# souravc83/Blackbox-Coresets-VI

Hardware: AMD Instinct MI355X
Metric: ELBO inner-steps/sec (S MC samples x M pseudopoints) at 1/2/4/8 GPU (higher is better)
Workload: dtype f32; 1 GPU; C3 fn2 full-cov MLP 64-40-40-2, S=128, M=100, one GPU (BASELINE configs[2]); S_total=128, M=100, D=64, H=40, C=2, params=4730326, parallelism=one GPU, adam=robust_higher DifferentiableAdam, elbo_finite=True

## Files before the change

### blackbox-coresets-vi_amd/csrc/capi.cpp

```cpp
#include <algorithm>
#include <cmath>
#include <cstdio>
#include <cstring>
#include <mutex>
#include <string>
#include <vector>

#include "psvi_diag.h"
#include "psvi_internal.hpp"

namespace psvi {
Diag g_diag;
}

using namespace psvi;

namespace {

thread_local std::string g_err;

int fail(int code, const std::string& msg) {
    g_err = msg;
    return code;
}
// ... 24 lines not shown
        if (d->dims[l] < 1) return fail(PSVI_EINVAL, "layer dims must be >= 1");
    if (d->S < 1) return fail(PSVI_EINVAL, "S must be >= 1");
    if (d->M < 1) return fail(PSVI_EINVAL, "M must be >= 1");
    if (!(d->prior_sd > 0.f)) return fail(PSVI_EINVAL, "prior_sd must be > 0");
    return 0;
}

int plan_to_device(psvi_plan& p) {
    const int S = p.d.S;
    const bool fullcov = p.family == PSVI_FAMILY_FULLCOV;
    if (int rc = upload(p.fwd)) return rc;
    if (int rc = upload(p.frb)) return rc;
    if (int rc = upload(p.upd)) return rc;
    if (p.fwd.n() > 0 && !p.fwd_part.alloc(sizeof(float) * (size_t)p.fwd.n() * S * kFwdRows))
        return fail(PSVI_EUNSUP, "cannot allocate the sample-phase scratch");
    if (p.fuse_sample && p.n_uslots > 0) {
        if (int rc = upload(p.ufrb)) return rc;
        if (!p.upd_part.alloc(sizeof(float) * (size_t)p.n_uslots * S * 64))
            return fail(PSVI_EUNSUP, "cannot allocate the fused-sample scratch");
    }
    if (p.str.n() > 0) {
        if (int rc = upload(p.str)) return rc;
        if (int rc = upload(p.sfrb)) return rc;
        const size_t nb = (size_t)std::max(1, p.sfrb.n());
        if (!p.str_part.alloc(sizeof(float) * (size_t)p.n_sslots * S * 64) ||
            !p.str_cnt.alloc(sizeof(int) * nb, true) || !p.str_bms.alloc(sizeof(float) * 128 * nb))
            return fail(PSVI_EUNSUP, "cannot allocate the streaming-update scratch");
    }
    if (p.n_kwg() > 0) {
        if (int rc = upload(p.ks_tiles)) return rc;
        if (int rc = upload(p.ks_segs)) return rc;
        if (int rc = upload(p.ks_off)) return rc;
        if (!p.ks_slots.alloc(sizeof(float) * (size_t)std::max(1, p.n_ks_slots) * kKsSlotFloats) ||
            !p.ks_cnt.alloc(sizeof(int) * std::max(1, p.n_ks_cnt), true))
            return fail(PSVI_EUNSUP, "cannot allocate the K-split update's slots");
    }
    if (p.n_fswg() > 0) {
        if (int rc = upload(p.fs_segs)) return rc;
        if (int rc = upload(p.fs_off)) return rc;
        if (int rc = upload(p.fs_rb)) return rc;
        if (int rc = upload(p.fp_segs)) return rc;
        if (int rc = upload(p.fp_off)) return rc;
        if (int rc = upload(p.fp_rb)) return rc;
        if (!p.fs_part.alloc(sizeof(float) * (size_t)std::max({1, p.n_fs_slots, p.n_fp_slots}) *
                             kKsPass * kFwdRows))
            return fail(PSVI_EUNSUP, "cannot allocate the segmented sample's slots");
    }
    if (fullcov) {
        net_xmap(p, p.xmap.host, p.net_bands.host);
        if (int rc = upload(p.xmap)) return rc;
        if (int rc = upload(p.net_bands)) return rc;
    }
    if (fullcov && p.mchunks > 1 &&
        !p.net_slots.alloc(sizeof(float) * (size_t)p.mchunks * std::max(1, p.s_cnt[p.rank]) * p.n_tot))
        return fail(PSVI_EUNSUP, "cannot allocate the network's pseudopoint-chunk slots");
    if (p.family == PSVI_FAMILY_MEANFIELD &&
        !p.mf_slots.alloc(sizeof(float) * (size_t)std::max(1, p.s_cnt[p.rank]) * p.mchunks * p.n_tot))
        return fail(PSVI_EUNSUP, "cannot allocate the mean-field gradient slots");
    if (fullcov && p.fuse_sample && p.tiles_total > 0 && !p.aux.create())
        return fail(PSVI_EUNSUP, "cannot create the inner loop's conversion stream");
    if (p.eps_planes_ok) {
        p.eps_planes_tab.host.assign(1, p.eps_planes);
        if (int rc = upload(p.eps_planes_tab)) return rc;
    }
    if (p.family == PSVI_FAMILY_LENET && !p.lenet_scratch.alloc(lenet_ws(p, nullptr).bytes))
        return fail(PSVI_EUNSUP, "cannot allocate the LeNet activation scratch");
    return 0;
}

hipStream_t as_stream(void* s) { return reinterpret_cast<hipStream_t>(s); }

int g_loop_every = 0;
std::vector<hipEvent_t> g_loop_ev[2];

void loop_events_clear() {
    for (auto& v : g_loop_ev) {
        for (hipEvent_t e : v) (void)hipEventDestroy(e);
        v.clear();
    }
}

hipError_t loop_event(int k, hipStream_t st) {
    hipEvent_t e;
    const hipError_t rc = hipEventCreate(&e);
    if (rc != hipSuccess) return rc;
    g_loop_ev[k].push_back(e);
    return hipEventRecord(e, st);
}

}

// ... 15 lines not shown
        case PSVI_DBG_FWD_ABLATION: g_diag.fwd_ablation = value; return 0;
        case PSVI_DBG_UPD_CHUNK: g_plan_dbg.upd_chunk_tiles = value; return 0;
        case PSVI_DBG_UPD_STREAM_OFF: g_diag.stream_off = value; return 0;
        case PSVI_DBG_STREAM_BF_OFF: g_diag.stream_bf_off = value; return 0;
        case PSVI_DBG_KSTREAM_OFF: g_diag.ks_off = value; return 0;
        case PSVI_DBG_KSTREAM_WGS: g_plan_dbg.ks_wgs = value; return 0;
        case PSVI_DBG_FWD_SEG_OFF: g_diag.fs_off = value; return 0;
        case PSVI_DBG_FWD_SEG_BF_OFF: g_diag.fs_bf_off = value; return 0;
        case PSVI_DBG_FWD_PAIR_BF: g_diag.fwd_pair_bf = value; return 0;
        case PSVI_DBG_STREAM_FOLD_OFF: g_diag.stream_fold_off = value; return 0;
        case PSVI_DBG_KSTREAM_BF_OFF: g_diag.ks_bf_off = value; return 0;
        case PSVI_DBG_ROP_VALU: g_diag.rop_valu = value; return 0;
        case PSVI_DBG_NET_SCALAR_LOADS: g_diag.net_scalar_loads = value; return 0;
        case PSVI_DBG_NET_MLOOP_OFF: g_diag.net_mloop_off = value; return 0;
        case PSVI_DBG_NET_GEO_OFF: g_diag.net_geo_off = value; return 0;
        case PSVI_DBG_NET_DRAW_SPARE_OFF: g_diag.net_draw_spare_off = value; return 0;
        case PSVI_DBG_NET_DRAW_ROLE1:
            if (value < 0 || value > 32) return fail(PSVI_EINVAL, "0..32");
            g_diag.net_draw_role1 = value;
            return 0;
        case PSVI_DBG_STREAM_WGS: g_plan_dbg.stream_wgs = value; return 0;
        case PSVI_DBG_STREAM_COST: g_plan_dbg.stream_cost = value; return 0;
        case PSVI_DBG_STREAM_RR: g_plan_dbg.stream_rr = value; return 0;
        case PSVI_DBG_LENET_ABLATION: g_diag.lenet_abl = value; return 0;
        case PSVI_DBG_NET_THREADS:
            if (value != 0 && value != 256 && value != 512) return fail(PSVI_EINVAL, "256 or 512");
            g_diag.net_threads = value;
            return 0;
        default: return fail(PSVI_EINVAL, "unknown debug key");
    }
}

int psvi_debug_loop_timing(double* out) {
    if (!out) return fail(PSVI_EINVAL, "null out");
    for (int k = 0; k < 2; ++k) {
        double sum = 0.0;
        const auto& v = g_loop_ev[k];
        for (size_t i = 0; i + 1 < v.size(); i += 2) {
            float ms = 0.f;
            HIP_TRY(hipEventSynchronize(v[i + 1]));
            HIP_TRY(hipEventElapsedTime(&ms, v[i], v[i + 1]));
            sum += ms;
        }
        const size_t n = v.size() / 2;
        out[k] = n ? 1e3 * sum / (double)n : 0.0;
        if (k == 0) out[2] = (double)n;
// ... 23 lines not shown
        return fail(PSVI_EINVAL, "unknown family");
    psvi_net_desc dl;
    if (family == PSVI_FAMILY_LENET && d) {
        dl = *d;
        dl.n_layers = 5;
        const int dims[6] = {784, 6, 16, 120, 84, 10};
        for (int l = 0; l < 6; ++l) dl.dims[l] = dims[l];
        d = &dl;
    }
    if (int rc = check_desc(d)) return rc;
    if (world < 1 || world > kMaxWorld || rank < 0 || rank >= world)
        return fail(PSVI_EINVAL, "world/rank out of range (world <= 8)");
    int ndev = 0;
    const bool have_dev = hipGetDeviceCount(&ndev) == hipSuccess && ndev > 0;
    if (have_dev) {
        static std::once_flag once;
        std::call_once(once, net_set_lds_limit);
    }
    psvi_plan* p = new psvi_plan();
    p->family = family;
    p->d = *d;
    p->world = world;
    p->rank = rank;
    std::string err;
    int rc = build_plan(*p, err);
    if (rc) rc = fail(rc, err);
    if (!rc && have_dev) {
        rc = plan_to_device(*p);
        p->on_device = rc == 0;
    }
    if (rc) {
        psvi_plan_destroy(p);
        return rc;
    }
    *out = p;
    return 0;
}

int psvi_plan_create_lik(int32_t family, const psvi_net_desc* d, int32_t world, int32_t rank,
                         const psvi_likelihood* lik, psvi_plan** out) {
    if (!lik || lik->kind == PSVI_LIK_CATEGORICAL)
        return psvi_plan_create(family, d, world, rank, out);
    if (!out) return fail(PSVI_EINVAL, "null out");
    *out = nullptr;
    if (lik->kind != PSVI_LIK_GAUSSIAN && lik->kind != PSVI_LIK_BERNOULLI)
        return fail(PSVI_EINVAL, "unknown likelihood kind");
// ... 1247 lines not shown
```

### blackbox-coresets-vi_amd/csrc/kernels_mvn_stream.hip

```cpp
#include "mvn_common.hpp"

namespace psvi {

struct StrArgs {
    const StreamRange* ranges;
    int nb[kMaxL];
    const float* eps;
    const float* eps_next;
    const float* g;
    int ldg, S;
    int64_t g_total, e_total;
    float* params;
    float* m;
    float* v;
    float* tp;
    float* tm;
    float* tv;
    float* part;
    double* kl_out;
    int include_kl;
    unsigned long long* stamps;
    float inv_s0sq, log_s0;
    AdamC adam;
    int xcol[kMaxL];
    MvnLayerArgs lay[kMaxL];
    const uint16_t* ep;
    const uint16_t* enp;
    int64_t pl;
// ... 44 lines not shown
        d = __builtin_elementwise_fma(sq, f32x2{a.inv_sqrt_bc2, a.inv_sqrt_bc2}, f32x2{a.eps, a.eps});
        const f32x2 r = {__builtin_amdgcn_rcpf(d[0]), __builtin_amdgcn_rcpf(d[1])};
        return p - (f32x2{a.lr_bc1, a.lr_bc1} * m) * r;
    } else {
        v = __builtin_elementwise_fma(b2, v, (omb2 * g) * g) + f32x2{1e-12f, 1e-12f};
        const f32x2 vb = v * f32x2{a.inv_bc2, a.inv_bc2};
        d = f32x2{__builtin_amdgcn_sqrtf(vb[0]), __builtin_amdgcn_sqrtf(vb[1])} + f32x2{a.eps, a.eps};
        const f32x2 r = {__builtin_amdgcn_rcpf(d[0]), __builtin_amdgcn_rcpf(d[1])};
        return p - f32x2{a.lr, a.lr} * (m * f32x2{a.inv_bc1, a.inv_bc1}) * r;
    }
}

template <int NS, int KIND, bool DIAG = false, bool SC1 = true, bool PAD = false>
__global__ __launch_bounds__(256, 1) void mvn_stream_kernel(StrArgs a) {
    constexpr int KT = 16 * NS;
    __shared__ __attribute__((aligned(16))) f32x4 sm[4 * kStrBuf + 2048];
    f32x4* const Gl4 = sm + 4 * kStrBuf;
    const float* const Gl = reinterpret_cast<const float*>(Gl4);
    const int tid = threadIdx.x, lane = tid & 63, wv = wave_id();
    const int wr = wv >> 1, wc = wv & 1, h = lane >> 5, l32 = lane & 31;
    const StreamRange R = a.ranges[blockIdx.x];
    const int t0 = __builtin_amdgcn_readfirstlane(R.t0);
    const int t1 = __builtin_amdgcn_readfirstlane(R.t1);
    int slot = __builtin_amdgcn_readfirstlane(R.slot0);
    const int S = a.S;
    unsigned long long tph[10] = {0, 0, 0, 0, 0, 0, 0, 0, 0, 0}, tlast = 0;
    auto ph = [&](int q) __attribute__((always_inline)) {
        if (DIAG && tid == 0) {
            const unsigned long long tt = __builtin_amdgcn_s_memtime();
            if (q >= 0) tph[q] += tt - tlast;
            tlast = tt;
        }
    };
    const int e_hi = PAD ? 0x7fffffff : (int)a.e_total - 4;
    const int g_hi = PAD ? 0x7fffffff : (int)a.g_total - 4;
    constexpr int SMAX = 32 * NS - 1;

    f32x4 ereg[8], enreg[8];
    auto load_E = [&](const StrTile& T) __attribute__((always_inline)) {
#pragma unroll
        for (int j = 0; j < 8; ++j) {
            const int f = tid + 256 * j, s = min(f >> 4, SMAX), c4 = f & 15;
            const int off = min(T.eoff + s * T.n + 64 * T.k + 4 * c4, e_hi);
            ereg[j] = *reinterpret_cast<const f32x4*>(a.eps + off);
            enreg[j] = *reinterpret_cast<const f32x4*>(a.eps_next + off);
        }
    };
// ... 66 lines not shown
#pragma unroll
        for (int q = 0; q < 16; ++q) xacc[sb][q] = 0.f;
    float klp = 0.f, kld = 0.f;
    f32x2 kl2 = {0.f, 0.f};

    int okd[8];
    {
        const int c = 32 * wc + l32, c4 = c >> 2;
#pragma unroll
        for (int k = 0; k < 8; ++k) okd[k] = h * 64 + 4 * ((c4 ^ h) ^ (2 * k)) + (c & 3);
    }
    int okx[4];
#pragma unroll
    for (int g = 0; g < 4; ++g) okx[g] = l32 * 16 + ((8 * wc + 2 * g + h) ^ (l32 & 15));
    const int ogb = h * 64 + 32 * wr + l32;

    if (DIAG && tid == 0) {
        a.stamps[(size_t)blockIdx.x * 16 + 12] = __builtin_amdgcn_s_memtime();
        a.stamps[(size_t)blockIdx.x * 16 + 13] = __builtin_amdgcn_s_memrealtime();
    }
    int tl = __builtin_amdgcn_readfirstlane(R.lbk0 >> 28);
    int tb_ = __builtin_amdgcn_readfirstlane((R.lbk0 >> 14) & 0x3fff);
    int tk = __builtin_amdgcn_readfirstlane(R.lbk0 & 0x3fff);
    StrTile cur = str_tile(a, tl, tb_, tk);
    load_E(cur);
    load_G(cur);
    store_E(0, cur);
    store_G(cur);
    __syncthreads();

    auto tile = [&](int i, const StrTile& nxt, auto has_next_c, auto newband_c) __attribute__((always_inline)) {
        constexpr bool has_next = decltype(has_next_c)::value;
        constexpr bool newband = decltype(newband_c)::value;
        const int bi = (i - t0) & 1;
        ph(-1);
        const float* Ef = reinterpret_cast<const float*>(sm + 2 * bi * kStrBuf);
        const f32x4* En = sm + (2 * bi + 1) * kStrBuf;
        load_pmv(cur);
        floatx16 acc;
#pragma unroll
        for (int q = 0; q < 16; ++q) acc[q] = 0.f;
#pragma unroll
        for (int t = 0; t < KT; ++t)
            acc = __builtin_amdgcn_mfma_f32_32x32x2f32(Ef[okd[t & 7] + 128 * t], Gl[ogb + 128 * t],
                                                       acc, 0, 0, 0);
        ph(0);
        const int n = cur.n, r = 64 * cur.b + 32 * wr + l32;
        if (cur.k == cur.b && wc == 0) {
            const int c = 32 * wr + l32;
            float pm2[2], ps2[2];
#pragma unroll
            for (int ww = 0; ww < 2; ++ww) {
                const int w = 2 * h + ww;
                float gm = 0.f, gsum = 0.f;
#pragma unroll
                for (int hh = 0; hh < (NS > 2 ? 2 : 1); ++hh)
#pragma unroll
// ... 106 lines not shown
#pragma unroll
                for (int q = 0; q < NLOAD; ++q)
                    if ((q * NSLOT) / (NLOAD > 0 ? NLOAD : 1) == k) issue_load(q);
                __builtin_amdgcn_sched_barrier(0x6);
            }
        }
        ph(2);
        ph(3);
        ph(4);
        if constexpr (has_next) store_E(bi ^ 1, nxt);
        ph(5);
        if constexpr (!has_next || newband) {
            __syncthreads();
            float* X = reinterpret_cast<float*>(sm + 2 * bi * kStrBuf);
            if (wc == 1) {
#pragma unroll
                for (int sb = 0; sb < NS; ++sb)
#pragma unroll
                    for (int q = 0; q < 16; ++q) X[((wr * NS + sb) * 16 + q) * 64 + lane] = xacc[sb][q];
            }
            if constexpr (newband) store_G(nxt);
            __syncthreads();
            if (wc == 0) {
                float* dst = a.part + (size_t)slot * S * 64 + 32 * wr + l32;
#pragma unroll
                for (int sb = 0; sb < NS; ++sb)
#pragma unroll
                    for (int q = 0; q < 16; ++q) {
                        const int s = 32 * sb + (q & 3) + 8 * (q >> 2) + 4 * h;
                        dst[(size_t)s * 64] = xacc[sb][q] + X[((wr * NS + sb) * 16 + q) * 64 + lane];
                    }
            }
#pragma unroll
            for (int sb = 0; sb < NS; ++sb)
#pragma unroll
                for (int q = 0; q < 16; ++q) xacc[sb][q] = 0.f;
            ++slot;
        }
        ph(6);
        __syncthreads();
        ph(7);
        if (DIAG && tid == 0) ++tph[9];
    };
    using T_ = std::true_type;
    using F_ = std::false_type;
    for (int i = t0; i + 1 < t1; ++i) {
        if (++tk > tb_) {
            tk = 0;
            int nbl = a.nb[0];
#pragma unroll
            for (int l = 1; l < kMaxL; ++l)
                if (tl == l) nbl = a.nb[l];
            if (++tb_ == nbl) {
                tb_ = 0;
                ++tl;
            }
        }
        const StrTile nxt = str_tile(a, tl, tb_, tk);
        if (nxt.l != cur.l || nxt.b != cur.b)
            tile(i, nxt, T_{}, T_{});
        else
            tile(i, nxt, T_{}, F_{});
        cur = nxt;
    }
    tile(t1 - 1, cur, F_{}, F_{});
    if (DIAG && tid == 0) {
        unsigned long long* o = a.stamps + (size_t)blockIdx.x * 16;
#pragma unroll
        for (int q = 0; q < 10; ++q) o[q] = tph[q];
        o[10] = __builtin_amdgcn_s_memtime();
        o[11] = __builtin_amdgcn_s_memrealtime();
    }
    klp = (klp + (kl2[0] + kl2[1])) * (0.5f * a.inv_s0sq) + kld;
    if (a.kl_out && a.include_kl) {
        const float tot = block_sum(klp, reinterpret_cast<float*>(sm));
        if (tid == 0) atomicAdd(a.kl_out, (double)tot);
    }
}


template <int KIND, bool DIAG = false, bool FOLD = false>
__global__ __launch_bounds__(512, 1) void mvn_stream_bf2_kernel(StrArgs a) {
    __shared__ __attribute__((aligned(16))) uint8_t smb[9 * kBfImg];
    uint8_t* const Eb = smb;
    uint8_t* const Gb = smb + 3 * kBfImg;
    uint8_t* const En = smb + 6 * kBfImg;
    float* const Xs = reinterpret_cast<float*>(En);
    float* const Xd = reinterpret_cast<float*>(Eb);
    uint32_t* const Xl = reinterpret_cast<uint32_t*>(Eb + 16384);
    float* const Xg = reinterpret_cast<float*>(Eb + 40960);
    typedef unsigned u32x4 __attribute__((ext_vector_type(4)));
    typedef unsigned u32x2 __attribute__((ext_vector_type(2)));
    const int tid = threadIdx.x, lane = tid & 63, wv = wave_id();
    const int q = wv & 3, hk = wv >> 2, wr = q >> 1, wc = q & 1, h = lane >> 5, l32 = lane & 31;
    const int pw = wv ^ 4;
    const StreamRange R = a.ranges[blockIdx.x];
    const int t0 = __builtin_amdgcn_readfirstlane(R.t0);
    const int t1 = __builtin_amdgcn_readfirstlane(R.t1);
    int slot = __builtin_amdgcn_readfirstlane(R.slot0);
    const int S = a.S;
    unsigned long long tph[11] = {0, 0, 0, 0, 0, 0, 0, 0, 0, 0, 0}, tlast = 0;
    if (DIAG && tid == 0) a.stamps[(size_t)blockIdx.x * 16 + 13] = __builtin_amdgcn_s_memtime();
    auto ph = [&](int qq) __attribute__((always_inline)) {
        if (DIAG && wv == 0) {
            const unsigned long long tt = __builtin_amdgcn_s_memtime();
            if (qq >= 0) tph[qq] += tt - tlast;
            tlast = tt;
        }
    };

    u32x4 stg[6];
    const int srow0 = tid >> 3, ch = tid & 7;
    const int st_col = srow0 * 128 + ((ch ^ (((srow0 >> 1) & 1) << 2)) << 4);
    const int st_row0 = img_row(srow0, 8 * ch), st_row1 = img_row(srow0, 8 * ch + 4);
    auto store_col = [&]() __attribute__((always_inline)) {
#pragma unroll
        for (int j = 0; j < 6; ++j)
            *reinterpret_cast<u32x4*>(Eb + st_col + (j >> 1) * kBfImg + 8192 * (j & 1)) = stg[j];
    };
    auto store_row = [&]() __attribute__((always_inline)) {
#pragma unroll
        for (int j = 0; j < 6; ++j) {
// ... 33 lines not shown
        return __builtin_bit_cast(u32x4, __builtin_amdgcn_raw_buffer_load_b128(r, vo, so, 0));
    };
    auto load_G = [&](const StrTile& T, int j) __attribute__((always_inline)) {
        const int so = __builtin_amdgcn_readfirstlane(4 * (32 * j * a.ldg + T.xc + 64 * T.b));
        greg[j] = __builtin_bit_cast(f32x4, ldb(rs_g, vo_g, so));
    };
    floatx16 xacc[2];
#pragma unroll
    for (int j = 0; j < 2; ++j)
#pragma unroll
        for (int qq = 0; qq < 16; ++qq) xacc[j][qq] = 0.f;
    float kld = 0.f;
    f32x2 kl2 = {0.f, 0.f};
    const int g16 = lane >> 4, qq4 = (lane >> 2) & 3, pp = lane & 3;
    const int ca = 32 * wc + 16 * (g16 & 1) + 4 * pp;
    const int cg = 32 * wr + 16 * (g16 & 1) + 4 * pp;
    const uint8_t* const rda = Eb + img_col(8 * h + qq4, ca);
    const uint8_t* const rdb = Gb + img_col(8 * h + qq4, cg);
    const int xsw = (l32 >> 1) & 7;

    int tl = __builtin_amdgcn_readfirstlane(R.lbk0 >> 28);
    int tb_ = __builtin_amdgcn_readfirstlane((R.lbk0 >> 14) & 0x3fff);
    int tk = __builtin_amdgcn_readfirstlane(R.lbk0 & 0x3fff);
    StrTile cur = str_tile(a, tl, tb_, tk);
    {
        const uint32_t vo = vo_planes(cur);
#pragma unroll
        for (int j = 0; j < 4; ++j) load_G(cur, j);
#pragma unroll
        for (int j = 0; j < 6; ++j) stg[j] = ldb(rs_e, vo, so_planes(cur, j));
        store_col();
#pragma unroll
        for (int j = 0; j < 6; ++j) stg[j] = ldb(rs_en, vo, so_planes(cur, j));
        store_row();
        split_G();
    }
    __syncthreads();

    auto issue_a = [&](int qi, const StrTile& nxt, bool has_next, uint32_t vo_n) __attribute__((always_inline)) {
        if (qi < 6) {
            const int gi = qi / 3, which = qi % 3;
            const int so = __builtin_amdgcn_readfirstlane((int)(cur.tb * 4));
            const u32x4 x = __builtin_bit_cast(
                u32x4, __builtin_amdgcn_raw_buffer_load_b128(rs_t, vo_f + 1024 * gi,
                                                             which == 0 ? so : which == 1 ? so + tmb : so + tvb,
                                                             PSVI_STATE_LOAD_AUX));
// ... 80 lines not shown
            }
#pragma unroll
            for (int i = 0; i < KR; ++i)
                if (k0 + i < nk)
#pragma unroll
                    for (int m = 0; m < 4; ++m) A[m][i & 3] += v[m][i];
        }
#pragma unroll
        for (int m = 0; m < 4; ++m) {
            const f32x4 t = (A[m][0] + A[m][1]) + (A[m][2] + A[m][3]);
            const int rr = 32 * (m >> 1) + lt;
            if (rr < R) {
#pragma unroll
                for (int e = 0; e < 4; ++e)
                    a.x[(int64_t)smp(m, e) * a.ldx + xcol + rr] =
                        (mu[m >> 1] + mul_unfused(dg[m >> 1], ev[m][e])) + t[e];
            }
        }
    };

    auto tile = [&](const StrTile& nxt, auto has_next_c, auto newband_c) __attribute__((always_inline)) {
        constexpr bool has_next = decltype(has_next_c)::value;
        constexpr bool newband = decltype(newband_c)::value;
        ph(-1);
        const bool diag = cur.k == cur.b && wc == wr;
        const uint32_t vo_n = vo_planes(nxt);
        floatx16 acc;
#pragma unroll
        for (int qq = 0; qq < 16; ++qq) acc[qq] = 0.f;
        float dgm = 0.f, dgs = 0.f;
        auto read_ab = [&](int t, bf8v (&av)[3], bf8v (&bv)[3]) __attribute__((always_inline)) {
#pragma unroll
            for (int p = 0; p < 3; ++p) {
                typedef __attribute__((address_space(3))) s4v* lds_s4;
                const int o = p * kBfImg + 2048 * t;
                av[p] = cat44(__builtin_amdgcn_ds_read_tr16_b64_v4i16((lds_s4)(rda + o)),
                              __builtin_amdgcn_ds_read_tr16_b64_v4i16((lds_s4)(rda + o + 512)));
                bv[p] = cat44(__builtin_amdgcn_ds_read_tr16_b64_v4i16((lds_s4)(rdb + o)),
                              __builtin_amdgcn_ds_read_tr16_b64_v4i16((lds_s4)(rdb + o + 512)));
            }
        };
#pragma unroll
        for (int t = 0; t < 4; ++t) {
            bf8v fa[3], fb[3];
            read_ab(4 * hk + t, fa, fb);
#pragma unroll
// ... 177 lines not shown
                            for (int e = 0; e < 4; ++e)
                                v4[e] = __float_as_uint(xacc[j][4 * qg + e] +
                                                        Xs[(((wr * 2 + hk) * 2 + j) * 16 + 4 * qg + e) * 64 + lane]);
                            BSTORE128(v4, rs_p, (uint32_t)((((((wr * 2 + hk) * 2 + j) * 4 + qg) * 64 + lane)) * 16),
                                      sob, 16);
                        }
                } else {
                    const uint32_t vb = (uint32_t)((32 * wr + l32 + 64 * (64 * hk + 4 * h)) * 4);
#pragma unroll
                    for (int j = 0; j < 2; ++j)
#pragma unroll
                        for (int qq = 0; qq < 16; ++qq) {
                            const int sl = 32 * j + (qq & 3) + 8 * (qq >> 2);
                            const float v = xacc[j][qq] + Xs[(((wr * 2 + hk) * 2 + j) * 16 + qq) * 64 + lane];
                            __builtin_amdgcn_raw_buffer_store_b32(__builtin_bit_cast(int, v), rs_p,
                                                                  vb + (uint32_t)(sl * 256), sob, 0);
                        }
                }
            }
#pragma unroll
            for (int j = 0; j < 2; ++j)
#pragma unroll
                for (int qq = 0; qq < 16; ++qq) xacc[j][qq] = 0.f;
            ++slot;
            if constexpr (FOLD) band_arrive();
        }
        ph(6);
        __syncthreads();
        ph(7);
        if constexpr (has_next) store_row();
        if constexpr (newband) {
            split_G();
            __syncthreads();
        }
        ph(8);
        if (DIAG && wv == 0) ++tph[9];
    };
    using T_ = std::true_type;
    using F_ = std::false_type;
    for (int i = t0; i + 1 < t1; ++i) {
        if (++tk > tb_) {
            tk = 0;
            int nbl = a.nb[0];
#pragma unroll
            for (int l = 1; l < kMaxL; ++l)
                if (tl == l) nbl = a.nb[l];
            if (++tb_ == nbl) {
                tb_ = 0;
                ++tl;
            }
        }
        const StrTile nxt = str_tile(a, tl, tb_, tk);
        if (nxt.l != cur.l || nxt.b != cur.b)
            tile(nxt, T_{}, T_{});
        else
            tile(nxt, T_{}, F_{});
        cur = nxt;
    }
    tile(cur, F_{}, F_{});
    if constexpr (FOLD) {
        ph(-1);
        for (int i = 0; i < nfold; ++i) band_combine(__builtin_amdgcn_readfirstlane(fold_list[i]));
        ph(10);
    }
    if (DIAG && tid == 0) {
        unsigned long long* o = a.stamps + (size_t)blockIdx.x * 16;
#pragma unroll
        for (int qq = 0; qq < 10; ++qq) o[qq] = tph[qq];
        o[10] = __builtin_amdgcn_s_memtime();
        o[11] = __builtin_amdgcn_s_memrealtime();
        o[12] = tph[10];
    }
// ... 14 lines not shown
    if (KIND == PSVI_ADAM_HIGHER && diag)
        hipLaunchKernelGGL((mvn_stream_kernel<4, PSVI_ADAM_HIGHER, true>), g, bl, 0, st, b);
    else if (pad)
        hipLaunchKernelGGL((mvn_stream_kernel<4, KIND, false, true, true>), g, bl, 0, st, b);
    else
        hipLaunchKernelGGL((mvn_stream_kernel<4, KIND>), g, bl, 0, st, b);
}
template <int KIND>
static void launch_stream_bf(bool diag, bool fold, dim3 g, hipStream_t st, const StrArgs& b) {
    const dim3 bl(512);
    if (KIND == PSVI_ADAM_HIGHER && diag && fold)
        hipLaunchKernelGGL((mvn_stream_bf2_kernel<PSVI_ADAM_HIGHER, true, true>), g, bl, 0, st, b);
    else if (fold)
        hipLaunchKernelGGL((mvn_stream_bf2_kernel<KIND, false, true>), g, bl, 0, st, b);
    else
        hipLaunchKernelGGL(mvn_stream_bf2_kernel<KIND>, g, bl, 0, st, b);
}

hipError_t launch_mvn_stream(const psvi_plan& p, const MvnUpdate& r, hipStream_t st) {
    StrArgs b{};
    fill_update(p, r, b);
    const int64_t tf = p.tiles_total * 4096;
    b.ranges = p.str.dev;
    b.eps_next = r.next.eps;
    b.tp = r.tstate;
    b.tm = r.tstate + tf;
    b.tv = r.tstate + 2 * tf;
    b.part = p.str_part.dev;
    for (int l = 0; l < p.L; ++l) {
        b.xcol[l] = p.xcol_l[p.rank][l];
        b.nb[l] = p.lay[l].nb;
    }
    const dim3 sg(p.str.n());
    const bool higher = b.adam.kind == PSVI_ADAM_HIGHER;
    const bool bf = r.eps_planes && r.next.planes && p.bf_stream && r.padded && !g_diag.stream_bf_off;
    if (bf) {
        b.stamps = g_diag.bf_stamps;
        b.ep = r.eps_planes;
        b.enp = r.next.planes;
        b.pl = p.eps_planes.pl;
        for (int l = 0; l < p.L; ++l) {
            b.ppoff[l] = p.eps_planes.poff[l];
            b.npad[l] = p.eps_planes.npad[l];
        }
        const bool fold = p.str_cnt.dev && p.str_bms.dev && p.str_max_ends <= kFoldMax && !g_diag.stream_fold_off;
        b.rbs = p.sfrb.dev;
// ... 17 lines not shown
```

### blackbox-coresets-vi_amd/csrc/plan_tables.cpp

```cpp
#include <algorithm>
#include <string>
#include <vector>

#include "psvi_internal.hpp"

namespace psvi {

PlanDebug g_plan_dbg;

namespace {

constexpr int kFwdKChunk = 256;
constexpr int64_t kLenetRowFloats = 2 * 1176 + 400 * 2 + 120 * 2 + 84 * 2 + 10;
constexpr int64_t kMaxOff = (int64_t(1) << 31) - 4096;

int fail(std::string& err, int code, const char* msg) {
    err = msg;
    return code;
}

std::vector<int64_t> cut_runs(const std::vector<double>& cum, int nwg) {
    const int64_t U = (int64_t)cum.size() - 1;
    std::vector<int64_t> cut(nwg + 1, 0);
    cut[nwg] = U;
// ... 131 lines not shown
            p.frb.host.push_back(
                FwdRowBlock{slot0, (int)fwd.size() - slot0, r1 - r0, xc + (r0 - lo), l, r0});
        }
        for (int b = lo / 64; 64 * b < hi; ++b) {
            const int slot0 = nslots;
            for (int k0 = 0; k0 <= b; k0 += ch) {
                const int k1 = std::min(b + 1, k0 + ch);
                upd.push_back(UpdChunk{l, 64 * b, k0, k1, lo, hi, xc - lo, k1 == b + 1, nslots++});
            }
            const int r0 = std::max(64 * b, lo), r1 = std::min(64 * b + 64, hi);
            p.ufrb.host.push_back(FwdRowBlock{slot0, nslots - slot0, r1 - r0, xc + (r0 - lo), l, r0});
        }
    }
    std::stable_sort(fwd.begin(), fwd.end(), [](const FwdItem& a, const FwdItem& b) {
        return (a.k1 - a.k0) > (b.k1 - b.k0);
    });
    p.upd.host = xcd_order(upd);
    p.n_uslots = nslots;
    p.upd_tiles = tiles;
}

void build_stream(psvi_plan& p) {
    const int r = p.rank;
    std::vector<uint32_t> tmap;
    std::vector<int> tband;
    int nband = 0;
    for (int l = 0; l < p.L; ++l)
        for (int b = 0; b < p.lay[l].nb; ++b, ++nband)
            for (int k = 0; k <= b; ++k) {
                tmap.push_back((uint32_t)l << 28 | (uint32_t)b << 14 | (uint32_t)k);
                tband.push_back(nband);
            }
    const int T = (int)tmap.size();
    const int nwg = std::max(1, std::min(g_plan_dbg.stream_wgs > 0 ? g_plan_dbg.stream_wgs : 256, T));
    const int cost = g_plan_dbg.stream_cost;
    std::vector<double> cum(T + 1, 0.0);
    for (int t = 0; t < T; ++t) {
        const uint32_t k = tmap[t] & 0x3fff, b = (tmap[t] >> 14) & 0x3fff;
        const double wd = cost >= 0 ? (cost / 1000) * 0.01 : 1.5;
        const double wf = cost >= 0 ? (cost % 1000) * 0.01 : 1.0;
        cum[t + 1] = cum[t] + 1.0 + (k == b ? wd : 0.0) + (k == 0 ? wf : 0.0);
    }
    const std::vector<int64_t> cut = cut_runs(cum, nwg);
    std::vector<StreamRange> runs;
    std::vector<std::vector<int>> band_slots(nband);
    int ns = 0;
    for (int w = 0; w < nwg; ++w) {
        const int t0 = (int)cut[w], t1 = (int)cut[w + 1];
        runs.push_back(StreamRange{t0, t1, ns, t0 < T ? tmap[t0] : 0u});
        int ends = 0;
        for (int t = t0; t < t1; ++t)
            if (t == t0 || tband[t] != tband[t - 1]) {
                band_slots[tband[t]].push_back(ns++);
                ++ends;
            }
        p.str_max_ends = std::max(p.str_max_ends, ends);
    }
    int bid = 0;
    for (int l = 0; l < p.L; ++l)
        for (int b = 0; b < p.lay[l].nb; ++b, ++bid) {
            const int r0 = 64 * b, R = std::min(64, p.lay[l].n - r0);
            const auto& sl = band_slots[bid];
            p.sfrb.host.push_back(
                FwdRowBlock{sl.front(), (int)sl.size(), R, p.xcol_l[r][l] + r0, l, r0});
        }
    for (int w = 0; w < nwg; ++w)
        p.str.host.push_back(runs[g_plan_dbg.stream_rr ? w : xcd_run(w, nwg)]);
    p.n_sslots = ns;
}

void build_kstream(psvi_plan& p) {
    const int r = p.rank, np = (p.d.S + kKsPass - 1) / kKsPass;
    std::vector<KsTile>& tiles = p.ks_tiles.host;
    tiles.clear();
    for (const ShardRun& run : p.runs[r])
        for (int b = run.lo / 64; 64 * b < run.hi; ++b)
            for (int k = 0; k <= b; ++k)
                tiles.push_back(KsTile{run.layer, 64 * b, k, k == b, 64 * b,
                                       std::min(64 * b + 64, p.lay[run.layer].n), run.col - run.lo, -1});
    const int T = (int)tiles.size();
    std::vector<KsSeg>& segs = p.ks_segs.host;
    std::vector<int>& off = p.ks_off.host;
    segs.clear();
    off.clear();
    p.n_ks_slots = p.n_ks_cnt = 0;
    if (T == 0) return;
    const int64_t U = (int64_t)T * np;
    int nwg = (int)std::min<int64_t>(U, g_plan_dbg.ks_wgs > 0 ? g_plan_dbg.ks_wgs : 512);
    if (nwg >= 8) nwg -= nwg % 8;
    std::vector<double> cum(U + 1, 0.0);
    for (int64_t u = 0; u < U; ++u) cum[u + 1] = cum[u] + 1.0 + (u % np == np - 1 ? 0.5 : 0.0);
// ... 225 lines not shown
```

### blackbox-coresets-vi_amd/csrc/psvi_diag.h

```cpp
#ifndef PSVI_DIAG_H
#define PSVI_DIAG_H
#include <stdint.h>

#ifdef __cplusplus
extern "C" {
#endif

#define PSVI_DBG_NET_ABLATION 1
int psvi_debug_set(int32_t key, int32_t value);
#define PSVI_DBG_NET_STAMPS 2
#define PSVI_DBG_UPD_ABLATION 3
#define PSVI_DBG_UPD_STAMPS 4
#define PSVI_DBG_NET_SPLIT_BELOW 5
#define PSVI_DBG_FWD_ABLATION 6
#define PSVI_DBG_FWD_STAMPS 7
int psvi_debug_set_ptr(int32_t key, void* ptr);
#define PSVI_DBG_LOOP_TIMING 8
#define PSVI_DBG_UPD_CHUNK 9
#define PSVI_DBG_UPD_STREAM_OFF 10
#define PSVI_DBG_STREAM_WGS 11
#define PSVI_DBG_STREAM_RR 12
#define PSVI_DBG_NET_THREADS 14
#define PSVI_DBG_NET_WG_TARGET 15
#define PSVI_DBG_LENET_ABLATION 17
#define PSVI_DBG_ROP_STAMPS 18
#define PSVI_DBG_KSTREAM_OFF 19
#define PSVI_DBG_NET_SCALAR_LOADS 20
#define PSVI_DBG_KSTREAM_WGS 21
#define PSVI_DBG_FWD_SEG_OFF 22
#define PSVI_DBG_NET_MLOOP_OFF 23
#define PSVI_DBG_STREAM_BF_OFF 24
#define PSVI_DBG_BF_STAMPS 25
#define PSVI_DBG_FWD_SEG_BF_OFF 26
#define PSVI_DBG_KSTREAM_BF_OFF 27
#define PSVI_DBG_ROP_VALU 29
#define PSVI_DBG_FWD_PAIR_BF 31
#define PSVI_DBG_NET_GEO_OFF 30
#define PSVI_DBG_STREAM_COST 34
#define PSVI_DBG_STREAM_FOLD_OFF 32
#define PSVI_DBG_NET_DRAW_PLANES 35
#define PSVI_DBG_NET_DRAW_ROLE1 36
#define PSVI_DBG_NET_DRAW_SPARE_OFF 37
int psvi_debug_loop_timing(double* out);


#ifdef __cplusplus
}
#endif
#endif
```

### blackbox-coresets-vi_amd/csrc/psvi_internal.hpp

```cpp
#pragma once
#include <hip/hip_runtime.h>
#include <stdint.h>

#include <algorithm>
#include <string>
#include <vector>

#include "psvi_hip.h"

namespace psvi {

constexpr int kMaxL = PSVI_MAX_LAYERS;
constexpr int kMaxWorld = 8;
constexpr int kWave = 64;

__device__ __forceinline__ float mul_unfused(float a, float b) {
    float r;
    asm("v_mul_f32 %0, %1, %2" : "=v"(r) : "v"(a), "v"(b));
    return r;
}
__device__ __forceinline__ float softplus_f(float x) {
    return x > 20.f ? x : log1pf(expf(x));
}
__device__ __forceinline__ float sigmoid_f(float x) { return 1.f / (1.f + expf(-x)); }
// ... 281 lines not shown
    int s0;
};
struct FsSeg {
    int layer, r0, r1, pass;
    int k0, k1, slot, pad;
};
struct UpdChunk {
    int layer, r0, k0, k1, rlo, rhi, xcol, diag;
    int slot;
};

struct KsTile {
    int layer, r0, k, diag;
    int rlo, rhi, xcol;
    int cnt;
};
constexpr int kKsPass = 128;
constexpr int kKsSlotFloats = 4096 + 512;
struct KsSeg {
    int tile, p0, p1;
    int slot, nc, ci;
};

struct StreamRange {
    int t0, t1, slot0;
    uint32_t lbk0;
};

struct ShardRun {
    int layer, lo, hi, col;
};

struct NetBand {
    int64_t base;
    int32_t stride, pad;
};

struct NetArgs;

struct NetOuter {
    int mode;
    int n_pseudo;
    float* nll_rows;
    const float* rowcoef;
    const float* ck;
    float* du_part;
    float* prob_rows;
    float* dz_part;
    bool loglik = false;
// ... 73 lines not shown
    int64_t Peps = 0;
    int n_tot = 0;
    int s_off[psvi::kMaxWorld], s_cnt[psvi::kMaxWorld];
    std::vector<psvi::ShardRun> runs[psvi::kMaxWorld];
    int rows_tot[psvi::kMaxWorld];
    int xcol_l[psvi::kMaxWorld][psvi::kMaxL];
    std::vector<int> band_owner, band_coloff;
    int band_base[psvi::kMaxL + 1] = {0};
    psvi::DevTable<uint32_t> xmap;
    psvi::DevTable<psvi::NetBand> net_bands;
    bool on_device = false;
    psvi::DevTable<psvi::FwdItem> fwd;
    psvi::DevTable<psvi::FwdRowBlock> frb;
    psvi::DevBuffer<float> fwd_part;
    psvi::DevTable<psvi::UpdChunk> upd;
    int upd_tiles = 0;
    bool fuse_sample = false;
    int64_t tiles_total = 0;
    psvi::DevTable<psvi::FwdRowBlock> ufrb;
    int n_uslots = 0;
    psvi::DevBuffer<float> upd_part;
    psvi::DevTable<psvi::StreamRange> str;
    psvi::DevTable<psvi::FwdRowBlock> sfrb;
    psvi::DevBuffer<float> str_part;
    psvi::DevBuffer<int> str_cnt;
    psvi::DevBuffer<float> str_bms;
    int str_max_ends = 0;
    int n_sslots = 0;
    psvi::DevTable<psvi::KsTile> ks_tiles;
    psvi::DevTable<psvi::KsSeg> ks_segs;
    psvi::DevTable<int> ks_off;
    psvi::DevBuffer<float> ks_slots;
    psvi::DevBuffer<int> ks_cnt;
    int n_ks_slots = 0, n_ks_cnt = 0;
    psvi::DevTable<psvi::FsSeg> fs_segs;
    psvi::DevTable<int> fs_off;
    psvi::DevTable<psvi::FwdRowBlock> fs_rb;
    psvi::DevBuffer<float> fs_part;
    int n_fs_slots = 0;
    psvi::DevTable<psvi::FsSeg> fp_segs;
    psvi::DevTable<int> fp_off;
    psvi::DevTable<psvi::FwdRowBlock> fp_rb;
    int n_fp_slots = 0;
    static int n_wg(const psvi::DevTable<int>& off) { return std::max(0, off.n() - 1); }
    int n_kwg() const { return n_wg(ks_off); }
    int n_fswg() const { return n_wg(fs_off); }
// ... 369 lines not shown
```

Measured before the change: 18160 inner-steps/s (one step: all S=128 samples x M=100 pseudopoints).

## Add column-panel traversal option for streaming full-covariance update tiles

```diff
diff --git a/blackbox-coresets-vi_amd/csrc/capi.cpp b/blackbox-coresets-vi_amd/csrc/capi.cpp
--- a/blackbox-coresets-vi_amd/csrc/capi.cpp
+++ b/blackbox-coresets-vi_amd/csrc/capi.cpp
@@ -70,6 +70,7 @@
     if (p.str.n() > 0) {
         if (int rc = upload(p.str)) return rc;
         if (int rc = upload(p.sfrb)) return rc;
+        if (int rc = upload(p.sseg)) return rc;
         const size_t nb = (size_t)std::max(1, p.sfrb.n());
         if (!p.str_part.alloc(sizeof(float) * (size_t)p.n_sslots * S * 64) ||
             !p.str_cnt.alloc(sizeof(int) * nb, true) || !p.str_bms.alloc(sizeof(float) * 128 * nb))
@@ -115,6 +116,8 @@
         return fail(PSVI_EUNSUP, "cannot allocate the LeNet activation scratch");
     return 0;
 }
+
+int g_stream_panel = kStreamPanelDefault;
 
 hipStream_t as_stream(void* s) { return reinterpret_cast<hipStream_t>(s); }
 
@@ -176,6 +179,10 @@
         case PSVI_DBG_STREAM_WGS: g_plan_dbg.stream_wgs = value; return 0;
         case PSVI_DBG_STREAM_COST: g_plan_dbg.stream_cost = value; return 0;
         case PSVI_DBG_STREAM_RR: g_plan_dbg.stream_rr = value; return 0;
+        case PSVI_DBG_STREAM_PANEL:
+            if (value < -1 || value > 0x4000) return fail(PSVI_EINVAL, "-1, or 0..16384 column blocks");
+            g_stream_panel = value < 0 ? kStreamPanelDefault : value;
+            return 0;
         case PSVI_DBG_LENET_ABLATION: g_diag.lenet_abl = value; return 0;
         case PSVI_DBG_NET_THREADS:
             if (value != 0 && value != 256 && value != 512) return fail(PSVI_EINVAL, "256 or 512");
@@ -245,6 +252,7 @@
     p->d = *d;
     p->world = world;
     p->rank = rank;
+    p->str_panel = g_stream_panel;
     std::string err;
     int rc = build_plan(*p, err);
     if (rc) rc = fail(rc, err);
diff --git a/blackbox-coresets-vi_amd/csrc/kernels_mvn_stream.hip b/blackbox-coresets-vi_amd/csrc/kernels_mvn_stream.hip
--- a/blackbox-coresets-vi_amd/csrc/kernels_mvn_stream.hip
+++ b/blackbox-coresets-vi_amd/csrc/kernels_mvn_stream.hip
@@ -4,6 +4,8 @@
 
 struct StrArgs {
     const StreamRange* ranges;
+    const int* sseg;
+    int panw;
     int nb[kMaxL];
     const float* eps;
     const float* eps_next;
@@ -94,7 +96,7 @@
     const StreamRange R = a.ranges[blockIdx.x];
     const int t0 = __builtin_amdgcn_readfirstlane(R.t0);
     const int t1 = __builtin_amdgcn_readfirstlane(R.t1);
-    int slot = __builtin_amdgcn_readfirstlane(R.slot0);
+    int seg = __builtin_amdgcn_readfirstlane(R.seg0);
     const int S = a.S;
     unsigned long long tph[10] = {0, 0, 0, 0, 0, 0, 0, 0, 0, 0}, tlast = 0;
     auto ph = [&](int q) __attribute__((always_inline)) {
@@ -207,6 +209,7 @@
     int tl = __builtin_amdgcn_readfirstlane(R.lbk0 >> 28);
     int tb_ = __builtin_amdgcn_readfirstlane((R.lbk0 >> 14) & 0x3fff);
     int tk = __builtin_amdgcn_readfirstlane(R.lbk0 & 0x3fff);
+    int pc0 = __builtin_amdgcn_readfirstlane(R.c0);
     StrTile cur = str_tile(a, tl, tb_, tk);
     load_E(cur);
     load_G(cur);
@@ -218,6 +221,8 @@
         constexpr bool has_next = decltype(has_next_c)::value;
         constexpr bool newband = decltype(newband_c)::value;
         const int bi = (i - t0) & 1;
+        int slot = 0;
+        if constexpr (!has_next || newband) slot = a.sseg[seg];
         ph(-1);
         const float* Ef = reinterpret_cast<const float*>(sm + 2 * bi * kStrBuf);
         const f32x4* En = sm + (2 * bi + 1) * kStrBuf;
@@ -370,7 +375,7 @@
             if constexpr (newband) store_G(nxt);
             __syncthreads();
             if (wc == 0) {
-                float* dst = a.part + (size_t)slot * S * 64 + 32 * wr + l32;
+                float* dst = a.part + (size_t)__builtin_amdgcn_readfirstlane(slot) * S * 64 + 32 * wr + l32;
 #pragma unroll
                 for (int sb = 0; sb < NS; ++sb)
 #pragma unroll
@@ -383,7 +388,7 @@
             for (int sb = 0; sb < NS; ++sb)
 #pragma unroll
                 for (int q = 0; q < 16; ++q) xacc[sb][q] = 0.f;
-            ++slot;
+            ++seg;
         }
         ph(6);
         __syncthreads();
@@ -393,15 +398,19 @@
     using T_ = std::true_type;
     using F_ = std::false_type;
     for (int i = t0; i + 1 < t1; ++i) {
-        if (++tk > tb_) {
-            tk = 0;
+        if (++tk > min(tb_, pc0 + a.panw - 1)) {
+            tk = pc0;
             int nbl = a.nb[0];
 #pragma unroll
             for (int l = 1; l < kMaxL; ++l)
                 if (tl == l) nbl = a.nb[l];
             if (++tb_ == nbl) {
-                tb_ = 0;
-                ++tl;
+                pc0 += a.panw;
+                if (pc0 >= nbl) {
+                    pc0 = 0;
+                    ++tl;
+                }
+                tb_ = tk = pc0;
             }
         }
         const StrTile nxt = str_tile(a, tl, tb_, tk);
@@ -445,7 +454,7 @@
     const StreamRange R = a.ranges[blockIdx.x];
     const int t0 = __builtin_amdgcn_readfirstlane(R.t0);
     const int t1 = __builtin_amdgcn_readfirstlane(R.t1);
-    int slot = __builtin_amdgcn_readfirstlane(R.slot0);
+    int seg = __builtin_amdgcn_readfirstlane(R.seg0);
     const int S = a.S;
     unsigned long long tph[11] = {0, 0, 0, 0, 0, 0, 0, 0, 0, 0, 0}, tlast = 0;
     if (DIAG && tid == 0) a.stamps[(size_t)blockIdx.x * 16 + 13] = __builtin_amdgcn_s_memtime();
@@ -525,6 +534,7 @@
     int tl = __builtin_amdgcn_readfirstlane(R.lbk0 >> 28);
     int tb_ = __builtin_amdgcn_readfirstlane((R.lbk0 >> 14) & 0x3fff);
     int tk = __builtin_amdgcn_readfirstlane(R.lbk0 & 0x3fff);
+    int pc0 = __builtin_amdgcn_readfirstlane(R.c0);
     StrTile cur = str_tile(a, tl, tb_, tk);
     {
         const uint32_t vo = vo_planes(cur);
@@ -651,6 +661,8 @@
     auto tile = [&](const StrTile& nxt, auto has_next_c, auto newband_c) __attribute__((always_inline)) {
         constexpr bool has_next = decltype(has_next_c)::value;
         constexpr bool newband = decltype(newband_c)::value;
+        int slot = 0;
+        if constexpr (!has_next || newband) slot = a.sseg[seg];
         ph(-1);
         const bool diag = cur.k == cur.b && wc == wr;
         const uint32_t vo_n = vo_planes(nxt);
@@ -874,7 +886,7 @@
             for (int j = 0; j < 2; ++j)
 #pragma unroll
                 for (int qq = 0; qq < 16; ++qq) xacc[j][qq] = 0.f;
-            ++slot;
+            ++seg;
             if constexpr (FOLD) band_arrive();
         }
         ph(6);
@@ -891,15 +903,19 @@
     using T_ = std::true_type;
     using F_ = std::false_type;
     for (int i = t0; i + 1 < t1; ++i) {
-        if (++tk > tb_) {
-            tk = 0;
+        if (++tk > min(tb_, pc0 + a.panw - 1)) {
+            tk = pc0;
             int nbl = a.nb[0];
 #pragma unroll
             for (int l = 1; l < kMaxL; ++l)
                 if (tl == l) nbl = a.nb[l];
             if (++tb_ == nbl) {
-                tb_ = 0;
-                ++tl;
+                pc0 += a.panw;
+                if (pc0 >= nbl) {
+                    pc0 = 0;
+                    ++tl;
+                }
+                tb_ = tk = pc0;
             }
         }
         const StrTile nxt = str_tile(a, tl, tb_, tk);
@@ -960,6 +976,8 @@
     fill_update(p, r, b);
     const int64_t tf = p.tiles_total * 4096;
     b.ranges = p.str.dev;
+    b.sseg = p.sseg.dev;
+    b.panw = p.str_panw;
     b.eps_next = r.next.eps;
     b.tp = r.tstate;
     b.tm = r.tstate + tf;
diff --git a/blackbox-coresets-vi_amd/csrc/plan_tables.cpp b/blackbox-coresets-vi_amd/csrc/plan_tables.cpp
--- a/blackbox-coresets-vi_amd/csrc/plan_tables.cpp
+++ b/blackbox-coresets-vi_amd/csrc/plan_tables.cpp
@@ -177,51 +177,57 @@
 
 void build_stream(psvi_plan& p) {
     const int r = p.rank;
+    const int W = p.str_panel > 0 ? std::min(p.str_panel, 0x4000) : 0x4000;
+    p.str_panw = W;
+    std::vector<int> bbase(p.L + 1, 0);
+    for (int l = 0; l < p.L; ++l) bbase[l + 1] = bbase[l] + p.lay[l].nb;
+    const int nband = bbase[p.L];
     std::vector<uint32_t> tmap;
-    std::vector<int> tband;
-    int nband = 0;
+    std::vector<int> tband, tc0;
     for (int l = 0; l < p.L; ++l)
-        for (int b = 0; b < p.lay[l].nb; ++b, ++nband)
-            for (int k = 0; k <= b; ++k) {
-                tmap.push_back((uint32_t)l << 28 | (uint32_t)b << 14 | (uint32_t)k);
-                tband.push_back(nband);
-            }
+        for (int c0 = 0; c0 < p.lay[l].nb; c0 += W)
+            for (int b = c0; b < p.lay[l].nb; ++b)
+                for (int k = c0; k <= std::min(b, c0 + W - 1); ++k) {
+                    tmap.push_back((uint32_t)l << 28 | (uint32_t)b << 14 | (uint32_t)k);
+                    tband.push_back(bbase[l] + b);
+                    tc0.push_back(c0);
+                }
     const int T = (int)tmap.size();
     const int nwg = std::max(1, std::min(g_plan_dbg.stream_wgs > 0 ? g_plan_dbg.stream_wgs : 256, T));
     const int cost = g_plan_dbg.stream_cost;
     std::vector<double> cum(T + 1, 0.0);
     for (int t = 0; t < T; ++t) {
         const uint32_t k = tmap[t] & 0x3fff, b = (tmap[t] >> 14) & 0x3fff;
+        const bool first = t == 0 || tband[t] != tband[t - 1];
         const double wd = cost >= 0 ? (cost / 1000) * 0.01 : 1.5;
         const double wf = cost >= 0 ? (cost % 1000) * 0.01 : 1.0;
-        cum[t + 1] = cum[t] + 1.0 + (k == b ? wd : 0.0) + (k == 0 ? wf : 0.0);
+        cum[t + 1] = cum[t] + 1.0 + (k == b ? wd : 0.0) + (first ? wf : 0.0);
     }
     const std::vector<int64_t> cut = cut_runs(cum, nwg);
+    std::vector<int> nseg(nband, 0), bslot(nband + 1, 0), seen(nband, 0);
+    for (int w = 0; w < nwg; ++w)
+        for (int t = (int)cut[w]; t < (int)cut[w + 1]; ++t)
+            if (t == (int)cut[w] || tband[t] != tband[t - 1]) ++nseg[tband[t]];
+    for (int i = 0; i < nband; ++i) bslot[i + 1] = bslot[i] + nseg[i];
     std::vector<StreamRange> runs;
-    std::vector<std::vector<int>> band_slots(nband);
-    int ns = 0;
+    std::vector<int>& sseg = p.sseg.host;
     for (int w = 0; w < nwg; ++w) {
-        const int t0 = (int)cut[w], t1 = (int)cut[w + 1];
-        runs.push_back(StreamRange{t0, t1, ns, t0 < T ? tmap[t0] : 0u});
-        int ends = 0;
+        const int t0 = (int)cut[w], t1 = (int)cut[w + 1], seg0 = (int)sseg.size();
         for (int t = t0; t < t1; ++t)
-            if (t == t0 || tband[t] != tband[t - 1]) {
-                band_slots[tband[t]].push_back(ns++);
-                ++ends;
-            }
+            if (t == t0 || tband[t] != tband[t - 1]) sseg.push_back(bslot[tband[t]] + seen[tband[t]]++);
+        const int ends = (int)sseg.size() - seg0;
+        runs.push_back(StreamRange{t0, t1, ends > 0 ? sseg[seg0] : 0, t0 < T ? tmap[t0] : 0u, seg0,
+                                   t0 < T ? tc0[t0] : 0, {0, 0}});
         p.str_max_ends = std::max(p.str_max_ends, ends);
     }
-    int bid = 0;
     for (int l = 0; l < p.L; ++l)
-        for (int b = 0; b < p.lay[l].nb; ++b, ++bid) {
-            const int r0 = 64 * b, R = std::min(64, p.lay[l].n - r0);
-            const auto& sl = band_slots[bid];
-            p.sfrb.host.push_back(
-                FwdRowBlock{sl.front(), (int)sl.size(), R, p.xcol_l[r][l] + r0, l, r0});
+        for (int b = 0; b < p.lay[l].nb; ++b) {
+            const int r0 = 64 * b, R = std::min(64, p.lay[l].n - r0), bid = bbase[l] + b;
+            p.sfrb.host.push_back(FwdRowBlock{bslot[bid], nseg[bid], R, p.xcol_l[r][l] + r0, l, r0});
         }
     for (int w = 0; w < nwg; ++w)
         p.str.host.push_back(runs[g_plan_dbg.stream_rr ? w : xcd_run(w, nwg)]);
-    p.n_sslots = ns;
+    p.n_sslots = bslot[nband];
 }
 
 void build_kstream(psvi_plan& p) {
diff --git a/blackbox-coresets-vi_amd/csrc/psvi_diag.h b/blackbox-coresets-vi_amd/csrc/psvi_diag.h
--- a/blackbox-coresets-vi_amd/csrc/psvi_diag.h
+++ b/blackbox-coresets-vi_amd/csrc/psvi_diag.h
@@ -37,6 +37,7 @@
 #define PSVI_DBG_FWD_PAIR_BF 31
 #define PSVI_DBG_NET_GEO_OFF 30
 #define PSVI_DBG_STREAM_COST 34
+#define PSVI_DBG_STREAM_PANEL 38
 #define PSVI_DBG_STREAM_FOLD_OFF 32
 #define PSVI_DBG_NET_DRAW_PLANES 35
 #define PSVI_DBG_NET_DRAW_ROLE1 36
diff --git a/blackbox-coresets-vi_amd/csrc/psvi_internal.hpp b/blackbox-coresets-vi_amd/csrc/psvi_internal.hpp
--- a/blackbox-coresets-vi_amd/csrc/psvi_internal.hpp
+++ b/blackbox-coresets-vi_amd/csrc/psvi_internal.hpp
@@ -327,9 +327,12 @@
     int slot, nc, ci;
 };
 
+constexpr int kStreamPanelDefault = 0;
 struct StreamRange {
     int t0, t1, slot0;
     uint32_t lbk0;
+    int seg0, c0;
+    int pad[2];
 };
 
 struct ShardRun {
@@ -449,6 +452,8 @@
     psvi::DevBuffer<float> upd_part;
     psvi::DevTable<psvi::StreamRange> str;
     psvi::DevTable<psvi::FwdRowBlock> sfrb;
+    psvi::DevTable<int> sseg;
+    int str_panel = 0, str_panw = 0;
     psvi::DevBuffer<float> str_part;
     psvi::DevBuffer<int> str_cnt;
     psvi::DevBuffer<float> str_bms;
```

Result: no change. 18130 inner-steps/s (one step: all S=128 samples x M=100 pseudopoints) (median of 2 runs) (-0.2%).
